# torognes/vsearch

Measured on AMD Instinct MI355X. Metric: GCUPS (useful DP cells/s of the search16 global-alignment path: DP + traceback + CIGAR), higher is better.
Workload: dtype int16

## Files before the change

include/vsx.h:

```cpp
#ifndef VSX_H
#define VSX_H

#include <stddef.h>
#include <stdint.h>

#ifdef __cplusplus
extern "C" {
#endif

#define VSX_API_VERSION 1000
#define VSX_SCORE_SENTINEL 32767

#define VSX_OK         0
#define VSX_EINVAL    -1
#define VSX_ENODEVICE -2
#define VSX_ENOMEM    -3
#define VSX_EHIP      -4

typedef struct vsx_ctx vsx_ctx;
typedef struct vsx_seqset vsx_seqset;
typedef struct vsx_plan vsx_plan;

typedef struct vsx_scoring {
  int64_t match;
// ... 47 lines not shown
  uint32_t traceback_launches;
  uint64_t cells;
  uint64_t dir_bytes;
} vsx_timing;

typedef struct vsx_plan_info {
  uint64_t tasks;
  uint64_t tasks_tilted;
  uint64_t tasks_tracked;
  uint32_t rows_dominant;
  uint32_t chunks;
  uint64_t tasks_max3;
  uint64_t tasks_sparse;
  uint64_t waves;
  uint64_t tasks_pair;
} vsx_plan_info;

const char * vsx_version_string(void);
int vsx_device_count(void);
const char * vsx_last_error(void);

int vsx_create(vsx_ctx ** out, const vsx_scoring * scoring, int device);
void vsx_destroy(vsx_ctx * ctx);


int vsx_seqset_create(vsx_ctx * ctx, vsx_seqset ** out, uint64_t n,
                      const char * blob, uint64_t blob_bytes,
                      const uint64_t * offsets, const uint32_t * lengths);
int vsx_seqset_create_from_device(vsx_ctx * ctx, vsx_seqset ** out, uint64_t n,
                                  const void * d_blob, uint64_t blob_bytes,
// ... 52 lines not shown
```

vsearch_amd/_lib.py:

```python
import ctypes as C
import os

HERE = os.path.dirname(os.path.abspath(__file__))
LIB_PATH = os.environ.get("VSX_LIBRARY") or os.path.join(HERE, "libvsx.so")

VSX_OK, VSX_EINVAL, VSX_ENODEVICE, VSX_ENOMEM, VSX_EHIP = 0, -1, -2, -3, -4
SENTINEL = 32767

SYMBOLS = [
    "vsx_version_string", "vsx_device_count", "vsx_last_error", "vsx_create", "vsx_destroy",
    "vsx_seqset_create", "vsx_seqset_create_both_strands", "vsx_seqset_create_from_device", "vsx_seqset_destroy", "vsx_seqset_count",
    "vsx_plan_create", "vsx_plan_run", "vsx_plan_sync", "vsx_plan_fetch", "vsx_plan_export_hits", "vsx_plan_export_runs",
    "vsx_cigar_from_runs", "vsx_plan_destroy",
    "vsx_align_pairs", "vsx_align_pairs_filtered", "vsx_align_pairs_ranked", "vsx_ranked_free", "vsx_plan_set_filter", "vsx_results_free", "vsx_plan_describe",
]
SEARCH_SYMBOLS = ["vsx_search_opts_default", "vsx_searcher_create", "vsx_searcher_destroy", "vsx_searcher_db_text", "vsx_search_batch",
                  "vsx_search_batch_meta", "vsx_searcher_set_meta",
                  "vsx_hits_free", "vsx_search_candidates", "vsx_search_candidates_batch", "vsx_candidates_free", "vsx_lma_align", "vsx_allpairs_block", "vsx_allpairs_rows", "vsx_allpairs_stream", "vsx_cluster_fast", "vsx_cluster_out_free", "vsx_msa", "vsx_msa_out_free",
                  "vsx_msa_device", "vsx_msa_device_batch", "vsx_dust_mask", "vsx_abundance_ratio_cmp",
                  "vsx_multi_searcher_create", "vsx_multi_searcher_destroy", "vsx_multi_searcher_devices", "vsx_multi_searcher_replica",
                  "vsx_multi_search_batch", "vsx_multi_allpairs",
                  "vsx_chimera_opts_default", "vsx_uchime_ref", "vsx_chimera_last_stats",
                  "vsx_chimera_denovo_opts_default", "vsx_uchime_denovo", "vsx_chimera_denovo_last_stats",
                  "vsx_chimeras_long_opts_default", "vsx_chimeras_denovo", "vsx_chimeras_denovo_last_stats",
# ... 191 lines not shown
                ("gaps", C.POINTER(C.c_uint16)), ("verdict", C.POINTER(C.c_uint8)), ("id", C.POINTER(C.c_double)),
                ("cigar_off", C.POINTER(C.c_uint64)), ("cigar_blob", C.POINTER(C.c_char)), ("cigar_bytes", C.c_uint64),
                ("n_undecided", C.c_uint64), ("undecided", C.POINTER(C.c_uint32))]


class Filter(C.Structure):
    _fields_ = [("iddef", C.c_int32), ("leftjust", C.c_int32), ("rightjust", C.c_int32), ("pad", C.c_int32),
                ("id", C.c_double), ("weak_id", C.c_double), ("maxid", C.c_double), ("mid", C.c_double),
                ("query_cov", C.c_double), ("target_cov", C.c_double),
                ("maxsubs", C.c_int64), ("maxgaps", C.c_int64), ("mincols", C.c_int64), ("maxdiffs", C.c_int64)]


class PlanInfo(C.Structure):
    _fields_ = [("tasks", C.c_uint64), ("tasks_tilted", C.c_uint64), ("tasks_tracked", C.c_uint64),
                ("rows_dominant", C.c_uint32), ("chunks", C.c_uint32), ("tasks_max3", C.c_uint64),
                ("tasks_sparse", C.c_uint64), ("waves", C.c_uint64), ("tasks_pair", C.c_uint64)]


class Timing(C.Structure):
    _fields_ = [("forward_ms", C.c_float), ("traceback_ms", C.c_float), ("total_ms", C.c_float),
                ("forward_launches", C.c_uint32), ("traceback_launches", C.c_uint32),
                ("cells", C.c_uint64), ("dir_bytes", C.c_uint64)]


class ClusterOut(C.Structure):
    _fields_ = [("n", C.c_uint64), ("n_clusters", C.c_uint64), ("clusterno", C.POINTER(C.c_uint32)), ("hits", Hits)]


class MsaOut(C.Structure):
    _fields_ = [("alnlen", C.c_uint64), ("n_rows", C.c_uint64), ("conslen", C.c_uint64), ("rows", C.POINTER(C.c_char)),
                ("consensus", C.POINTER(C.c_char)), ("profile", C.POINTER(C.c_uint64))]
# ... 125 lines not shown
```

vsearch_amd/csrc/ubench_d16.hip:

```cpp
#include <hip/hip_runtime.h>
#include <cstdio>
#include <cstdlib>

#define CK(x) do { hipError_t e = (x); if (e != hipSuccess) { fprintf(stderr, "%s:%d %s\n", __FILE__, __LINE__, hipGetErrorString(e)); exit(1); } } while (0)

__global__ void k_semantics(unsigned * out)
{
  __shared__ unsigned short tab[256];
  tab[threadIdx.x] = (unsigned short) (0x1100u + threadIdx.x);
  tab[threadIdx.x + 64] = (unsigned short) (0x2200u + threadIdx.x);
  __syncthreads();
  const unsigned addr = (unsigned) (size_t) tab + threadIdx.x * 2u;
  unsigned hi = 0xDEADBEEFu, lo = 0xDEADBEEFu, u16 = 0xDEADBEEFu;
  asm volatile("ds_read_u16_d16_hi %0, %3 offset:128\n"
               "ds_read_u16_d16 %1, %3\n"
               "ds_read_u16 %2, %3\n"
               "s_waitcnt lgkmcnt(0)\n" : "+v"(hi), "+v"(lo), "+v"(u16) : "v"(addr));
  out[threadIdx.x * 3 + 0] = hi;
  out[threadIdx.x * 3 + 1] = lo;
  out[threadIdx.x * 3 + 2] = u16;
}

typedef _Float16 f16x2 __attribute__((ext_vector_type(2)));
typedef unsigned short us2 __attribute__((ext_vector_type(2)));
// ... 53 lines not shown
        uint4 v4 = make_uint4(0, 0, 0, 0);
#pragma unroll
        for (int r = 0; r < R; ++r)
          {
            if ((r & 3) == 0) v4 = q4[r >> 2];
            const unsigned V = (r & 3) == 0 ? v4.x : ((r & 3) == 1 ? v4.y : ((r & 3) == 2 ? v4.z : v4.w));
            const unsigned h0 = Hd + V;
            const unsigned h2 = max3(h0, F, E[r]);
            Hd = hin[r];
            hout[r] = h2;
            const unsigned he = h2 - go;
            F = pmaxu(F, he);
            E[r] = pmaxu(E[r], he);
          }
      }
    else
      {
        const unsigned aA = (unsigned) (size_t) QP + (ca * (16 * R) + (unsigned) l * R) * 2u;
        const unsigned aB = (unsigned) (size_t) QP + (cb * (16 * R) + (unsigned) l * R) * 2u;
        unsigned lo[R], hi[R];
#define LOAD2(k) asm volatile("ds_read_u16 %0, %4 offset:%6\n ds_read_u16_d16_hi %1, %5 offset:%6\n ds_read_u16 %2, %4 offset:%7\n ds_read_u16_d16_hi %3, %5 offset:%7\n" \
                              : "=&v"(lo[2 * (k)]), "=&v"(hi[2 * (k)]), "=&v"(lo[2 * (k) + 1]), "=&v"(hi[2 * (k) + 1]) : "v"(aA), "v"(aB), "n"(4 * (k)), "n"(4 * (k) + 2))
#define WAIT2(k, n) asm volatile("s_waitcnt lgkmcnt(" #n ")" : "+v"(lo[2 * (k)]), "+v"(hi[2 * (k)]), "+v"(lo[2 * (k) + 1]), "+v"(hi[2 * (k) + 1]))
        LOAD2(0); LOAD2(1);
#pragma unroll
        for (int k = 0; k < R / 2; ++k)
          {
            if (k + 1 < R / 2) { WAIT2(k, 4); } else { WAIT2(k, 0); }
#pragma unroll
            for (int rr = 0; rr < 2; ++rr)
// ... 25 lines not shown
{
  const int blocks = 1024 * waves_per_simd, steps = 2000;
  unsigned * out; CK(hipMalloc(&out, (size_t) blocks * 64 * 4));
  hipEvent_t e0, e1; CK(hipEventCreate(&e0)); CK(hipEventCreate(&e1));
  hipLaunchKernelGGL(k_rows<MODE>, dim3(blocks), dim3(64), 0, 0, 20, out, 1u);
  CK(hipDeviceSynchronize());
  CK(hipEventRecord(e0));
  hipLaunchKernelGGL(k_rows<MODE>, dim3(blocks), dim3(64), 0, 0, steps, out, 1u);
  CK(hipEventRecord(e1));
  CK(hipEventSynchronize(e1));
  float ms; CK(hipEventElapsedTime(&ms, e0, e1));
  unsigned h0 = 0;
  CK(hipMemcpy(&h0, out, 4, hipMemcpyDeviceToHost));
  const double cycles = ms * 1e-3 * 2.4e9;
  printf("mode %d (%s) waves/SIMD %d: %8.3f ms, %.1f cycles per lane-row and wave   [check %08x]\n", MODE,
         MODE == 0 ? "b64 loads + perm, 6 VALU per row" : (MODE == 1 ? "u16 loads, add3, 5 VALU per row" : "pair profile, b128 loads, 5 VALU per row"), waves_per_simd, ms,
         cycles / ((double) steps * R * waves_per_simd), h0);
  CK(hipFree(out));
}

int main()
{
  hipDeviceProp_t p; CK(hipGetDeviceProperties(&p, 0));
  printf("device %s  CUs %d  arch %s\n", p.name, p.multiProcessorCount, p.gcnArchName);
  unsigned * out; CK(hipMalloc(&out, 64 * 3 * 4));
  hipLaunchKernelGGL(k_semantics, dim3(1), dim3(64), 0, 0, out);
  unsigned h[12]; CK(hipMemcpy(h, out, sizeof h, hipMemcpyDeviceToHost));
  printf("lane 0: d16_hi into 0xDEADBEEF -> %08x, d16 -> %08x, u16 -> %08x;  lane 1: %08x %08x %08x\n", h[0], h[1], h[2], h[3], h[4], h[5]);
  printf("  (table: lane x holds 0x1100 + x at its address, 0x2200 + x at +128)  d16_hi zeroes the low half: %s\n", (h[0] & 0xffffu) == 0 ? "YES" : "no");
  for (int w = 1; w <= 4; w *= 2) { run<0>(w); run<1>(w); if (w <= 2) run<2>(w); }
  run<0>(3);
  return 0;
}
```

vsearch_amd/csrc/vsx_device.hip:

```cpp
#include <hip/hip_runtime.h>
#include <type_traits>
#include <cstdlib>
#include <atomic>
#include "vsx_internal.h"

typedef unsigned int u32;
typedef unsigned int u32x4 __attribute__((ext_vector_type(4)));
typedef unsigned int u32x3 __attribute__((ext_vector_type(3)));
typedef short s2 __attribute__((ext_vector_type(2)));
typedef unsigned short us2 __attribute__((ext_vector_type(2)));

#define DEV __device__ __forceinline__
struct __attribute__((aligned(4))) Pair2 { unsigned int x, y; };

#define SIGN2 0x80008000u

DEV s2 S2(u32 x) { return __builtin_bit_cast(s2, x); }
DEV us2 U2(u32 x) { return __builtin_bit_cast(us2, x); }
DEV u32 UI(s2 x) { return __builtin_bit_cast(u32, x); }
DEV u32 UI(us2 x) { return __builtin_bit_cast(u32, x); }

DEV u32 sadd(u32 a, u32 b) { return UI(__builtin_elementwise_add_sat(S2(a), S2(b))); }
DEV u32 ssub(u32 a, u32 b) { return UI(__builtin_elementwise_sub_sat(S2(a), S2(b))); }
DEV u32 pmax(u32 a, u32 b) { return UI(__builtin_elementwise_max(S2(a), S2(b))); }
// ... 30 lines not shown
#ifndef VSX_FWD_WAVES
#define VSX_FWD_WAVES(R_, TILT_) ((R_) <= 16 ? 4 : ((R_) <= 24 ? 3 : 2))
#endif
#ifndef VSX_FWD_WAVES_ONE
#define VSX_FWD_WAVES_ONE(R_, TILT_) ((R_) == 26 ? 3 : VSX_FWD_WAVES(R_, TILT_))
#endif
typedef _Float16 f16x2 __attribute__((ext_vector_type(2)));
DEV u32 pk_max3_bits(u32 a, u32 b, u32 c)
{
  const f16x2 x = __builtin_bit_cast(f16x2, a), y = __builtin_bit_cast(f16x2, b), z = __builtin_bit_cast(f16x2, c);
  return __builtin_bit_cast(u32, __builtin_elementwise_maximum(__builtin_elementwise_maximum(x, y), z));
}
#ifndef VSX_FWD_WAVES_NQ
#define VSX_FWD_WAVES_NQ(R_, NQ_) ((NQ_) == 4 ? 2 : ((R_) <= 24 ? 3 : 2))
#endif
template <int R, bool TRACK, bool TILT = false, bool MAX3 = false, int NQ = 1, bool PAIR = false, bool ONE = false>
__global__ void __launch_bounds__(PAIR ? 256 : 64) __attribute__((amdgpu_waves_per_eu(NQ == 1 ? (ONE ? VSX_FWD_WAVES_ONE(R, TILT) : VSX_FWD_WAVES(R, TILT)) : VSX_FWD_WAVES_NQ(R, NQ), 8)))
vsx_forward_kernel(const VsxDevParams P, const VsxTask * __restrict__ tasks,
                   const uint8_t * __restrict__ qc, const uint8_t * __restrict__ tc,
                   u32 * __restrict__ dir, uint2 * strip, VsxSlotOut * __restrict__ slot_out, const u32 ntasks)
{
  constexpr bool TOPPAD = !TRACK;
  static_assert(!TILT || TOPPAD, "tilted coordinates exist for the TOPPAD class only");
  const int tl = TILT ? P.tilt : 0;
  static_assert(!MAX3 || TILT, "the MAX3 arithmetic is a sub-class of TILT");
  constexpr u32 BIAS16 = MAX3 ? 0x3E00u : (TILT ? 0x8000u : 0u);
  constexpr u32 BIAS = BIAS16 * 0x10001u;
  constexpr u32 CK_REBIAS = 0u;
  auto bpack = [](int v) -> u32 { return pack16(v + (int) BIAS16); };
  auto vadd = [](u32 a, u32 b) -> u32 { return TILT ? a + b : sadd(a, b); };
  auto vsubk = [](u32 a, u32 b) -> u32 { return TILT ? a - b : ssub(a, b); };
  auto vsub = [](u32 a, u32 b) -> u32 { return TILT ? psubw(a, b) : ssub(a, b); };
  auto vmax = [](u32 a, u32 b) -> u32 { return TILT ? pmaxu(a, b) : pmax(a, b); };
  constexpr bool MIDCK = VSX_MID(R, TILT);
  constexpr int RT = MIDCK ? R / 2 : R;
  constexpr bool QPL = TILT;
  constexpr int RP = (R + 3) & ~3;
  static_assert(NQ == 1 || NQ == 2 || NQ == 4, "tasks per wave");
  static_assert(NQ == 1 || TILT, "the sparse-task classes exist for the look-ahead TILT kernels only");
  static_assert(!PAIR || (NQ == 1 && TILT), "the pair-profile classes extend the FEED2 look-ahead kernels");
  constexpr int WPB = PAIR ? 4 : 1;
  constexpr int QPBYTES = 16 * 16 * RP;
  constexpr int RPP = ((RP / 4) & 1) ? RP : RP + 4;
  __shared__ __attribute__((aligned(16))) u32 PPf[PAIR ? 16 * 16 * RPP : 4];
  __shared__ __attribute__((aligned(16))) int16_t QP[!PAIR ? (QPL ? (NQ * QPBYTES) / 2 : 16 * 16 * R) : 8];
  constexpr int FSZ = (TILT ? 2 : 1) * 4 * 16;
  __shared__ uint4 FEED4a[FSZ * WPB];
  __shared__ u32 FEEDFa[FSZ * WPB];
  constexpr bool FEED2 = TILT;
  __shared__ uint2 FEEDBa[FEED2 ? 2 * 4 * 16 * WPB : 1];

  const int wv = PAIR ? __builtin_amdgcn_readfirstlane((int) (threadIdx.x >> 6)) : 0;
  uint4 * const FEED4 = FEED4a + wv * FSZ;
  u32 * const FEEDF = FEEDFa + wv * FSZ;
  uint2 * const FEEDB = FEEDBa + (FEED2 ? wv * FSZ : 0);
  const int lane = PAIR ? (int) (threadIdx.x & 63) : (int) threadIdx.x;
  const int gw = lane >> 4;
  constexpr int GPT = 4 / NQ;
  const int sq = (NQ == 1) ? 0 : gw / GPT;
  const int g = (NQ == 1) ? gw : gw % GPT;
  const int l = lane & 15;
  const u32 tix = PAIR ? blockIdx.x * 4u + (u32) wv : ((NQ == 1) ? blockIdx.x : blockIdx.x * (u32) NQ + (u32) sq);
  const bool sub_on = (NQ == 1 && !PAIR) ? true : (tix < ntasks);
  const VsxTask & T = tasks[sub_on ? tix : ntasks - 1];
  uint8_t * const QPl = reinterpret_cast<uint8_t *>(QP) + ((NQ == 1) ? 0 : sq * QPBYTES);

  const int Q = (int) T.qlen;
  const int total_lanes = (Q + R - 1) / R;
  const int rcnt0 = Q - (total_lanes - 1) * R;
  const int rc0 = __builtin_amdgcn_readfirstlane(rcnt0);
// ... 34 lines not shown
                  int va = 0, vb = 0;
                  if (rr < R)
                    {
                      if (Lr == 0 && rr < pad) va = vb = -P.top_step + 2 * tl;
                      else if (Lr < total_lanes)
                        {
                          const int gi = (Lr == 0) ? rr - pad : rcnt0 + (Lr - 1) * R + rr;
                          const int qs = (int) qq[gi];
                          va = P.matrix[(1 << (pr >> 2)) * 16 + qs];
                          vb = P.matrix[(1 << (pr & 3)) * 16 + qs];
                        }
                    }
                  PPf[(pr * 16 + row / RP) * RPP + rr] = ((u32) va & 0xffu) | (((u32) vb & 0xffu) << 16);
                }
            }
          else if (QPL)
            {
              constexpr int LPT = 64 / NQ;
              for (int idx = (NQ == 1) ? lane : lane % LPT; idx < 16 * 16 * RP; idx += LPT)
                {
                  const int code = idx / (16 * RP), row = idx % (16 * RP);
                  const int Lr = 16 * s + row / RP, rr = row % RP;
                  int v = 0;
                  if (rr < R)
                    {
                      if (Lr == 0 && rr < pad) v = -P.top_step + 2 * tl;
                      else if (Lr < total_lanes)
                        {
                          const int gi = (Lr == 0) ? rr - pad : rcnt0 + (Lr - 1) * R + rr;
                          v = P.matrix[code * 16 + (int) qq[gi]];
// ... 62 lines not shown
        rawA = (c < DA) ? (u32) tA[c] : 0u;
        rawB = (c < DB) ? (u32) tB[c] : 0u;
        if (s == 0) rawH = P.htop[c];
        else if (c < Dpg) rawS = strip_in[c];
      };
      prefetch(0);

      auto build_feed = [&](int blk, auto lean_tag) __attribute__((always_inline)) {
              constexpr bool LEAN = FEED2 && decltype(lean_tag)::value;
              const int c = 16 * blk + l;
              if (LEAN)
                {
                  f_H = (s == 0) ? bpack(rawH - pad * tl) : rawS.x;
                  f_F = (s == 0) ? vsub(f_H, qrt_i_pk) : rawS.y;
                  const u32 f_off = PAIR ? (((rawA >> 1) - (rawA >> 3)) * 4u + ((rawB >> 1) - (rawB >> 3))) * (u32) (16 * RPP * 4)
                                         : (rawA * (u32) (16 * RP) | ((rawB * (u32) (16 * RP)) << 16));
                  FEED4[(blk & 1) * 64 + gw * 16 + l] = make_uint4(f_off, 0u, f_H, f_F);
                  prefetch(blk + 1);
                  return;
                }
              const u32 qA = (u32) ((c < DA - 1) ? P.qrt_i : P.qrt_r) & 0xffffu;
              const u32 qB = (u32) ((c < DB - 1) ? P.qrt_i : P.qrt_r) & 0xffffu;
              const u32 rA = (u32) ((c < DA - 1) ? P.rt_i : P.rt_r) & 0xffffu;
              const u32 rB = (u32) ((c < DB - 1) ? P.rt_i : P.rt_r) & 0xffffu;
              const u32 sA = rawA | ((c == DA - 1) ? 0x100u : 0u) | ((c < DpA) ? 0x200u : 0u);
              const u32 sB = rawB | ((c == DB - 1) ? 0x100u : 0u) | ((c < DpB) ? 0x200u : 0u);
              f_sym = sA | (sB << 16);
              f_qrt = qA | (qB << 16);
              f_rt = rA | (rB << 16);
              if (s == 0)
                {
                  f_H = bpack(rawH - pad * tl);
                  f_F = vsub(f_H, f_qrt);
                }
              else
                {
                  f_H = rawS.x;
                  f_F = rawS.y;
                }
              const int fo = QPL ? (blk & 1) * 64 : 0;
              if (FEED2)
                {
                  const u32 f_off = PAIR ? (((rawA >> 1) - (rawA >> 3)) * 4u + ((rawB >> 1) - (rawB >> 3))) * (u32) (16 * RPP * 4)
                                         : (rawA * (u32) (16 * RP) | ((rawB * (u32) (16 * RP)) << 16));
                  FEED4[fo + gw * 16 + l] = make_uint4(f_off, f_sym, f_H, f_F);
                  FEEDB[fo + gw * 16 + l] = make_uint2(f_qrt, f_rt);
                }
              else
                {
                  FEED4[fo + gw * 16 + l] = make_uint4(f_sym, f_qrt, f_rt, f_H);
                  FEEDF[fo + gw * 16 + l] = f_F;
                }
              prefetch(blk + 1);
      };
      constexpr int PD = RP / 4;
      u32 profA[2][(QPL && !PAIR) ? PD : 1], profB[2][(QPL && !PAIR) ? PD : 1];
      auto load_profile = [&](u32 (&buf)[2][(QPL && !PAIR) ? PD : 1], u32 sy) __attribute__((always_inline)) {
        if (PAIR) return;
        const u32 cd = sy & 0x000F000Fu;
        constexpr int QPA = (RP % 16 == 0) ? 16 : ((RP % 8 == 0) ? 8 : 4);
        if (FEED2)
          {
            const uint8_t * pa = QPl + l * RP + (sy & 0xFFFFu);
            const uint8_t * pb = QPl + l * RP + (sy >> 16);
            constexpr int PDN = (QPL && !PAIR) ? PD : 1;
            if constexpr (PAIR) { }
            else if constexpr (QPA == 16)
              {
#pragma unroll
                for (int k = 0; k < PDN; k += 4)
                  {
                    const uint4 va = *reinterpret_cast<const uint4 *>(pa + 4 * k), vb = *reinterpret_cast<const uint4 *>(pb + 4 * k);
                    buf[0][k] = va.x; buf[0][k + 1] = va.y; buf[0][k + 2] = va.z; buf[0][k + 3] = va.w;
// ... 11 lines not shown
                  }
              }
            else
              {
#pragma unroll
                for (int k = 0; k < PDN; ++k)
                  { buf[0][k] = reinterpret_cast<const u32 *>(pa)[k]; buf[1][k] = reinterpret_cast<const u32 *>(pb)[k]; }
              }
            return;
          }
        const u32 * a = reinterpret_cast<const u32 *>(QPl + (cd & 0xFu) * (16 * RP) + l * RP);
        const u32 * b = reinterpret_cast<const u32 *>(QPl + (cd >> 16) * (16 * RP) + l * RP);
#pragma unroll
        for (int k = 0; k < ((QPL && !PAIR) ? PD : 1); ++k) { buf[0][k] = a[k]; buf[1][k] = b[k]; }
      };
      if (QPL)
        {
          build_feed(0, std::false_type {});
          sym = dpp_shr1(FEED4[gw * 16].x, 0u);
          load_profile(profA, sym);
        }

      const uint4 * const feed4_g = FEED4 + gw * 16;
      const u32 * const feedf_g = FEEDF + gw * 16;
      u32 pendH = 0, pendF = 0;
      u32 pendMH = 0, pendMF = 0, curMH = 0, curMF = 0;
      bool pend_on = false;
      const size_t ck_rowdw = ((((size_t) nstrips * steps + 1) & ~(size_t) 1) >> 1) * VSX_ROWCK_PAIR_DW(TILT);
      const size_t ck_nblk = ((size_t) steps + 15) >> 4;
      constexpr int CK_LANE_DW = TILT ? 3 : 4;
      constexpr size_t CK_COL_DW = TILT ? (size_t) 64 * 4 * VSX_COLCK_NB(R, true) : (size_t) 64 * (2 * R);
      const int ck_slot = VSX_CK_SLOT(TILT, gw, l);
      u32 * const rck_base = dir + T.dir_off + ((((size_t) s * steps) >> 1) * 64 + ck_slot) * CK_LANE_DW;
      u32 * const cck_base = dir + T.dir_off + ck_rowdw + (size_t) s * ck_nblk * CK_COL_DW;
      u32 * const mck_base = dir + T.dir_off + ck_rowdw + (size_t) nstrips * ck_nblk * CK_COL_DW
// ... 19 lines not shown
            }
          if (QPL) { if ((t & 15) == 15) build_feed((t >> 4) + 1, std::integral_constant<bool, LEANFEED> {}); }
          else if ((t & 15) == 0) build_feed(t >> 4, std::false_type {});

          const int fo = QPL ? ((t >> 4) & 1) * 64 : 0;
          const u32 fslot = (u32) (fo + (t & 15));
          const uint4 fv = feed4_g[fslot];
          const u32 fF = FEED2 ? fv.w : feedf_g[fslot];
          if (QPL)
            {
              const int t1 = t + 1;
              symn = dpp_shr1(feed4_g[(u32) (((t1 >> 4) & 1) * 64 + (t1 & 15))].x, sym);
              load_profile(pn, symn);
            }
          else sym = dpp_shr1(fv.x, sym);
          if (!INTERIOR)
            {
              if (FEED2)
                {
                  const uint2 fb = FEEDB[fo + gw * 16 + (t & 15)];
                  qrt = dpp_shr1(fb.x, qrt); rt = dpp_shr1(fb.y, rt);
                  symf = dpp_shr1(fv.y, symf);
                }
              else { qrt = dpp_shr1(fv.y, qrt); rt = dpp_shr1(fv.z, rt); }
            }
          const u32 inH = dpp_shr1(FEED2 ? fv.z : fv.w, outH);
          const u32 inF = dpp_shr1(fF, outF);

          const int j = t - l;
          const bool active = STEADY ? true : (lane_on && j >= 0 && j < Dpg);
          if (active)
            {
              const u32 code = sym & 0x000F000Fu;
              const int16_t * qpA = QP + (code & 0xFu) * (16 * R) + l * R;
              const int16_t * qpB = QP + (code >> 16) * (16 * R) + l * R;
              u32 pa = 0, pb = 0;
              u32 Hd = diag;
              u32 F = inF;
              u32 smn = 0x7FFF7FFFu, smx = 0x80008000u;
              u32 h2 = 0;
              u32 capH = 0, capF = 0, capmn = 0, capmx = 0;
              u32 lastL = 0, lastEL = 0;
              u32 midH = 0, midF = 0;
              auto rows = [&](auto shared_tag) __attribute__((always_inline)) {
              constexpr bool SHARED = decltype(shared_tag)::value;
              constexpr bool LASTFAST = MAX3 && SHARED;
#pragma unroll
              for (int r = 0; r < R; ++r)
                {
                  u32 V;
                  if (PAIR) V = pp[r];
                  else if (QPL)
                    {
                      if ((r & 3) == 0) { pa = pc[0][r >> 2]; pb = pc[1][r >> 2]; }
                      V = __builtin_amdgcn_perm(pb, pa, 0x0C040C00u + 0x00010001u * (u32) (r & 3));
                    }
                  else
                    {
                      if (R % 2 == 0)
                        {
                          if ((r & 3) == 0 && r + 3 < R)
                            {
                              typedef typename std::conditional<R % 4 == 0, uint2, Pair2>::type Rows4;
                              const Rows4 va = *reinterpret_cast<const Rows4 *>(qpA + r);
                              const Rows4 vb = *reinterpret_cast<const Rows4 *>(qpB + r);
                              pa = va.x; pb = vb.x;
                              ac[r + 1] = va.y; ac[r + 2] = vb.y;
                            }
                          else if ((r & 3) == 0)
                            {
                              pa = *reinterpret_cast<const u32 *>(qpA + r);
                              pb = *reinterpret_cast<const u32 *>(qpB + r);
                            }
                          else if ((r & 3) == 2) { pa = ac[r - 1]; pb = ac[r]; }
                          V = (r & 1) ? __builtin_amdgcn_perm(pb, pa, 0x07060302u) : __builtin_amdgcn_perm(pb, pa, 0x05040100u);
                        }
                      else V = (u32) (uint16_t) qpA[r] | ((u32) (uint16_t) qpB[r] << 16);
                    }
                  const u32 h0 = vadd(Hd, V);
                  const bool ONE_MAX = MAX3 && (r < R - 1 || LASTFAST);
                  const u32 h1 = ONE_MAX ? 0u : vmax(h0, F);
                  h2 = ONE_MAX ? pk_max3_bits(h0, F, E[r]) : vmax(h1, E[r]);
                  if (TRACK) { smn = pmin(smn, h2); smx = pmax(smx, h2); }
                  Hd = hin[r];
                  hout[r] = h2;
                  const u32 qrq = (r == R - 1) ? qrq_last : P.qrq_i_pk;
                  const u32 rq = (r == R - 1) ? rq_last : P.rq_i_pk;
                  const u32 he = (r < R - 1) ? vsubk(h2, qrq) : vsub(h2, qrq);
                  const u32 hf = (SHARED && r < R - 1) ? he : vsub(h2, qrt);
                  const u32 f = (TILT && INTERIOR) ? F : vsub(F, rt);
                  const u32 e = (TILT && INTERIOR && r < R - 1) ? E[r] : vsub(E[r], rq);
                  if (r == R - 1) { lastL = LASTFAST ? 0u : vsub(h1, E[r]); lastEL = vsub(he, e); }
                  F = vmax(f, hf);
                  E[r] = vmax(e, he);
// ... 1400 lines not shown
static hipError_t launch_fwd2(int track, int nq, int one, const VsxDevParams & P, const VsxTask * d_tasks, uint32_t ntasks,
                              const uint8_t * q, const uint8_t * t, uint32_t * dir, uint2 * strip,
                              VsxSlotOut * slot, hipStream_t st)
{
  if (nq == 8)
    {
      if (!(P.tilt != 0 && !track) || (ntasks & 3u)) return hipErrorInvalidValue;
      if constexpr (R >= 4)
        {
          if (!one) return hipErrorInvalidValue;
          if (P.max3) VSX_FWD_GO4(ntasks / 4, R, false, true, true, 1, true, true); else VSX_FWD_GO4(ntasks / 4, R, false, true, false, 1, true, true);
          return hipGetLastError();
        }
      else return hipErrorInvalidValue;
    }
  if (nq != 1)
    {
      if (!(P.tilt != 0 && !track && (nq == 2 || nq == 4))) return hipErrorInvalidValue;
      if constexpr (R >= 4)
        {
          const uint32_t grid = (ntasks + (uint32_t) nq - 1) / (uint32_t) nq;
          if (nq == 2) { if (P.max3) VSX_FWD_GO(grid, R, false, true, true, 2); else VSX_FWD_GO(grid, R, false, true, false, 2); }
          else         { if (P.max3) VSX_FWD_GO(grid, R, false, true, true, 4); else VSX_FWD_GO(grid, R, false, true, false, 4); }
          return hipGetLastError();
        }
      else return hipErrorInvalidValue;
    }
  if (P.tilt != 0)
    {
      if (track) return hipErrorInvalidValue;
// ... 95 lines not shown
```

vsearch_amd/csrc/vsx_host.cpp:

```cpp
#include "../../include/vsx.h"
#include "vsx_internal.h"
#include "vsx_private.h"

#include <hip/hip_runtime.h>
#include <algorithm>
#include <cinttypes>
#include <cstdio>
#include <cstdlib>
#include <cstring>
#include <sched.h>
#include <thread>
#include <atomic>
#include <condition_variable>
#include <mutex>
#include <chrono>
#include <deque>
#include <functional>
#include <memory>
#include <numeric>
#include <string>
#include <vector>

using vsxp::fail;
using vsxp::DevBuf;
// ... 885 lines not shown
  {
    std::vector<uint64_t> bad((size_t) nthc, UINT64_MAX);
    auto check = [&](int t) {
      const uint64_t lo = n_pairs * (uint64_t) t / (uint64_t) nthc, hi = n_pairs * (uint64_t) (t + 1) / (uint64_t) nthc;
      for (uint64_t k = lo; k < hi; ++k)
        if (qidx[k] >= queries->n || tidx[k] >= targets->n) { bad[(size_t) t] = k; return; }
    };
    run_threads(nthc, check);
    for (int t = 0; t < nthc; ++t)
      if (bad[(size_t) t] != UINT64_MAX)
        return fail(VSX_EINVAL, "vsx_plan_create: pair %" PRIu64 " references a sequence out of range", bad[(size_t) t]);
  }
  VSX_HIP(hipSetDevice(ctx->device));
  static const bool pair_env = std::getenv("VSX_PAIRPROF") ? std::strcmp(std::getenv("VSX_PAIRPROF"), "0") != 0 : (VSX_PAIRPROF_DEFAULT != 0);
  const bool pair_try = pair_env && n_pairs >= 32;

  std::unique_ptr<vsx_plan> pl(new vsx_plan);
  pl->ctx = ctx; pl->Q = queries; pl->T = targets; pl->n_pairs = n_pairs;
  {
    std::lock_guard<std::mutex> lk(ctx->slot_mu);
    const unsigned seq = ctx->plan_seq.fetch_add(1);
    int pick = -1;
    for (int k = 0; k < 3; ++k)
      if (ctx->slot_refs[k] == 0 && (pick < 0 || ctx->shared_dir[k].bytes() > ctx->shared_dir[pick].bytes())) pick = k;
    if (pick < 0)
      for (int k = 0; k < 3; ++k)
        if (pick < 0 || (int) (seq - ctx->slot_stamp[k]) > (int) (seq - ctx->slot_stamp[pick])) pick = k;
    ++ctx->slot_refs[pick];
    ctx->slot_stamp[pick] = seq;
    pl->dir_slot = pick;
// ... 205 lines not shown
      std::vector<Key> ks;
      for (const ProtoTask & pt : protos)
        {
          if (pt.nq != 2 && pt.nq != 4) continue;
          bool found = false;
          for (Key & c : ks) if (c.rows == pt.rows && c.track == pt.track && c.tilt == pt.tilt && c.nq == pt.nq) { ++c.count; found = true; break; }
          if (!found) ks.push_back(Key {pt.rows, pt.track, pt.tilt, pt.nq, 1});
        }
      bool any = false;
      for (const Key & c : ks) any = any || c.count < sparse_min;
      if (any)
        for (ProtoTask & pt : protos)
          if (pt.nq == 2 || pt.nq == 4)
            for (const Key & c : ks)
              if (c.count < sparse_min && pt.nq == c.nq && pt.rows == c.rows && pt.track == c.track && pt.tilt == c.tilt) { pt.nq = 1; break; }
    }
  auto by_class = [](const ProtoTask & a, const ProtoTask & b) {
    if (a.rows != b.rows) return a.rows < b.rows;
    if (a.track != b.track) return a.track < b.track;
    if (a.tilt != b.tilt) return a.tilt < b.tilt;
    return a.nq < b.nq;
  };
  if (!std::is_sorted(protos.begin(), protos.end(), by_class)) std::stable_sort(protos.begin(), protos.end(), by_class);

  double t_budget = 0;
  if (dir_budget_bytes == 0)
    {
      size_t free_b = 0, total_b = 0;
      const double tb0 = now();
      VSX_HIP(hipMemGetInfo(&free_b, &total_b));
// ... 248 lines not shown
  VSX_HIP(hipMemsetAsync(pl->d_cursor.p, 0, 2 * sizeof(unsigned long long), st));
  if (pl->filter.rank_counts) VSX_HIP(hipMemsetAsync(pl->d_rank_counts.p, 0, 2 * sizeof(uint32_t), st));
  VSX_HIP(hipEventRecord(pl->ev_begin, st));
  for (size_t k = 0; k < pl->chunks.size(); ++k)
    {
      Chunk & c = pl->chunks[k];
      uint32_t * dir = pl->d_dir[0].p;
      if (k >= 1) VSX_HIP(hipStreamWaitEvent(st, pl->chunks[k - 1].e2, 0));
      else if (ctx->ev_tb_used[slot]) VSX_HIP(hipStreamWaitEvent(st, ctx->ev_tb[slot], 0));
      VSX_HIP(hipEventRecord(c.e0, st));
      for (const Launch & L : c.launches)
        {
          VsxDevParams Pf = L.tilt ? ctx->Pt : ctx->P;
          Pf.max3 = (L.tilt == 2) ? 1 : 0;
          static const bool one_off = std::getenv("VSX_ONESTRIP") && std::strcmp(std::getenv("VSX_ONESTRIP"), "0") == 0;
          VSX_HIP(vsx_launch_forward(L.rows, L.track, L.nq, (L.multi || (one_off && L.nq != 8)) ? 0 : 1, Pf, pl->d_tasks.p + L.first, L.count,
                                    pl->Q->codes(), pl->T->codes(), dir, pl->d_strip.p,
                                    pl->d_slot.p + (size_t) L.first * VSX_TASK_SLOTS, st));
        }
      VSX_HIP(hipEventRecord(c.e1, st));
      VSX_HIP(hipStreamWaitEvent(st2, c.e1, 0));
      VSX_HIP(hipEventRecord(c.e1b, st2));
      for (size_t li = 0; li < c.launches.size();)
        {
          const Launch & L = c.launches[li];
          uint32_t pair_count = L.pair_count;
          size_t lj = li + 1;
          while (lj < c.launches.size() && c.launches[lj].rows == L.rows &&
                 c.launches[lj].track == L.track && c.launches[lj].tilt == L.tilt) { pair_count += c.launches[lj].pair_count; ++lj; }
          VsxDevParams Pb = L.tilt ? ctx->Pt : ctx->P;
          Pb.max3 = (L.tilt == 2) ? 1 : 0;
// ... 43 lines not shown
  return VSX_OK;
}

int vsx_plan_describe(const vsx_plan * pl, vsx_plan_info * info)
{
  if (!pl || !info) return fail(VSX_EINVAL, "vsx_plan_describe: null argument");
  *info = vsx_plan_info {};
  info->tasks = pl->tasks.size();
  info->chunks = (uint32_t) pl->chunks.size();
  uint64_t best = 0;
  for (const Chunk & c : pl->chunks)
    for (const Launch & L : c.launches)
      {
        if (L.nq == 2 || L.nq == 4) info->tasks_sparse += L.count;
        if (L.nq == 8) info->tasks_pair += L.count;
        info->waves += (L.nq == 2 || L.nq == 4) ? (L.count + (uint32_t) L.nq - 1) / (uint32_t) L.nq : L.count;
        if (L.tilt) info->tasks_tilted += L.count;
        if (L.tilt == 2) info->tasks_max3 += L.count;
        if (L.track) info->tasks_tracked += L.count;
        if (L.count > best) { best = L.count; info->rows_dominant = (uint32_t) L.rows; }
      }
  return VSX_OK;
}

static void append_cigar(std::string & s, const uint32_t * runs, uint32_t n)
{
  static const char ops[4] = {'M', 'I', 'D', '?'};
  char buf[16];
  for (uint32_t k = n; k-- > 0;)
    {
// ... 547 lines not shown
```

vsearch_amd/csrc/vsx_internal.h:

```cpp
#ifndef VSX_INTERNAL_H
#define VSX_INTERNAL_H

#include <stdint.h>
#include <hip/hip_runtime_api.h>

#define VSX_TASK_SLOTS 8
#define VSX_GROUP_LANES 16
#define VSX_MAX_SEQLEN_SUM 65535LL
#define VSX_MAX_SEQLEN_PRODUCT 25000000LL
#define VSX_TABLE_LEN (65536 + 64)
#define VSX_CODE_SLACK 64
#define VSX_CK_SLACK_DW 4096
#ifndef VSX_MID_MIN_ROWS
#define VSX_MID_MIN_ROWS 18
#endif
#define VSX_MID(R_, TILT_) ((TILT_) && (R_) >= VSX_MID_MIN_ROWS)

struct VsxDevParams {
  uint32_t match_pk;
  uint32_t qrq_i_pk, rq_i_pk;
  uint32_t qrq_r_pk, rq_r_pk;
  int32_t  qrt_i, rt_i;
  int32_t  qrt_r, rt_r;
  int32_t  match, mismatch;
  int32_t  smin;
  int32_t  n_mismatch;
  int32_t  share_sub;
  int32_t  top_open, top_step;
  int32_t  tilt;
  int32_t  max3;
  const int16_t * htop;
// ... 166 lines not shown
```

Measured before the change: 8208.

## Add split LO/HI query-profile forward kernel class for pure MAX3 single-strip tasks

```diff
diff --git a/include/vsx.h b/include/vsx.h
--- a/include/vsx.h
+++ b/include/vsx.h
@@ -85,6 +85,7 @@
   uint64_t tasks_sparse;
   uint64_t waves;
   uint64_t tasks_pair;
+  uint64_t tasks_split;
 } vsx_plan_info;
 
 const char * vsx_version_string(void);
diff --git a/vsearch_amd/_lib.py b/vsearch_amd/_lib.py
--- a/vsearch_amd/_lib.py
+++ b/vsearch_amd/_lib.py
@@ -229,7 +229,8 @@
 class PlanInfo(C.Structure):
     _fields_ = [("tasks", C.c_uint64), ("tasks_tilted", C.c_uint64), ("tasks_tracked", C.c_uint64),
                 ("rows_dominant", C.c_uint32), ("chunks", C.c_uint32), ("tasks_max3", C.c_uint64),
-                ("tasks_sparse", C.c_uint64), ("waves", C.c_uint64), ("tasks_pair", C.c_uint64)]
+                ("tasks_sparse", C.c_uint64), ("waves", C.c_uint64), ("tasks_pair", C.c_uint64),
+                ("tasks_split", C.c_uint64)]
 
 
 class Timing(C.Structure):
diff --git a/vsearch_amd/csrc/ubench_d16.hip b/vsearch_amd/csrc/ubench_d16.hip
--- a/vsearch_amd/csrc/ubench_d16.hip
+++ b/vsearch_amd/csrc/ubench_d16.hip
@@ -91,6 +91,34 @@
             E[r] = pmaxu(E[r], he);
           }
       }
+    else if (MODE == 3)
+      {
+        const char * base = reinterpret_cast<const char *>(QP) + l * 16;
+        const char * pa = base + (ca & 3u) * 1024u, * pb = base + ((cb & 3u) + 4u) * 1024u;
+        uint4 lo = *reinterpret_cast<const uint4 *>(pa), hi = *reinterpret_cast<const uint4 *>(pb), lo2, hi2;
+#pragma unroll
+        for (int r = 0; r < R; ++r)
+          {
+            if ((r & 3) == 0)
+              {
+                if (r) { lo = lo2; hi = hi2; }
+                const int k = (r >> 2) + 1;
+                if (k < R / 4) { lo2 = *reinterpret_cast<const uint4 *>(pa + k * 256); hi2 = *reinterpret_cast<const uint4 *>(pb + k * 256); }
+                else { lo2 = *reinterpret_cast<const uint4 *>(base + (cb & 3u) * 1024u); hi2 = *reinterpret_cast<const uint4 *>(base + ((ca & 3u) + 4u) * 1024u); }
+              }
+            const unsigned vl = (r & 3) == 0 ? lo.x : ((r & 3) == 1 ? lo.y : ((r & 3) == 2 ? lo.z : lo.w));
+            const unsigned vh = (r & 3) == 0 ? hi.x : ((r & 3) == 1 ? hi.y : ((r & 3) == 2 ? hi.z : hi.w));
+            const unsigned h0 = Hd + vl + vh;
+            const unsigned h2 = max3(h0, F, E[r]);
+            Hd = hin[r];
+            hout[r] = h2;
+            const unsigned he = h2 - go;
+            F = pmaxu(F, he);
+            E[r] = pmaxu(E[r], he);
+          }
+        Hd ^= lo2.x & hi2.x & 1u;
+        diag ^= Hd & 1u;
+      }
     else
       {
         const unsigned aA = (unsigned) (size_t) QP + (ca * (16 * R) + (unsigned) l * R) * 2u;
@@ -146,7 +174,7 @@
   CK(hipMemcpy(&h0, out, 4, hipMemcpyDeviceToHost));
   const double cycles = ms * 1e-3 * 2.4e9;
   printf("mode %d (%s) waves/SIMD %d: %8.3f ms, %.1f cycles per lane-row and wave   [check %08x]\n", MODE,
-         MODE == 0 ? "b64 loads + perm, 6 VALU per row" : (MODE == 1 ? "u16 loads, add3, 5 VALU per row" : "pair profile, b128 loads, 5 VALU per row"), waves_per_simd, ms,
+         MODE == 0 ? "b64 loads + perm, 6 VALU per row" : (MODE == 1 ? "u16 loads, add3, 5 VALU per row" : (MODE == 2 ? "pair profile, b128 loads, 5 VALU per row" : "split LO / HI tables, 2 x b128 per 4 rows, add3, 5 VALU per row")), waves_per_simd, ms,
          cycles / ((double) steps * R * waves_per_simd), h0);
   CK(hipFree(out));
 }
@@ -162,5 +190,6 @@
   printf("  (table: lane x holds 0x1100 + x at its address, 0x2200 + x at +128)  d16_hi zeroes the low half: %s\n", (h[0] & 0xffffu) == 0 ? "YES" : "no");
   for (int w = 1; w <= 4; w *= 2) { run<0>(w); run<1>(w); if (w <= 2) run<2>(w); }
   run<0>(3);
+  run<3>(4); run<3>(3);
   return 0;
 }
diff --git a/vsearch_amd/csrc/vsx_device.hip b/vsearch_amd/csrc/vsx_device.hip
--- a/vsearch_amd/csrc/vsx_device.hip
+++ b/vsearch_amd/csrc/vsx_device.hip
@@ -68,7 +68,7 @@
 #ifndef VSX_FWD_WAVES_NQ
 #define VSX_FWD_WAVES_NQ(R_, NQ_) ((NQ_) == 4 ? 2 : ((R_) <= 24 ? 3 : 2))
 #endif
-template <int R, bool TRACK, bool TILT = false, bool MAX3 = false, int NQ = 1, bool PAIR = false, bool ONE = false>
+template <int R, bool TRACK, bool TILT = false, bool MAX3 = false, int NQ = 1, bool PAIR = false, bool ONE = false, bool SPLIT = false>
 __global__ void __launch_bounds__(PAIR ? 256 : 64) __attribute__((amdgpu_waves_per_eu(NQ == 1 ? (ONE ? VSX_FWD_WAVES_ONE(R, TILT) : VSX_FWD_WAVES(R, TILT)) : VSX_FWD_WAVES_NQ(R, NQ), 8)))
 vsx_forward_kernel(const VsxDevParams P, const VsxTask * __restrict__ tasks,
                    const uint8_t * __restrict__ qc, const uint8_t * __restrict__ tc,
@@ -93,21 +93,25 @@
   static_assert(NQ == 1 || NQ == 2 || NQ == 4, "tasks per wave");
   static_assert(NQ == 1 || TILT, "the sparse-task classes exist for the look-ahead TILT kernels only");
   static_assert(!PAIR || (NQ == 1 && TILT), "the pair-profile classes extend the FEED2 look-ahead kernels");
+  static_assert(!SPLIT || (TILT && MAX3 && NQ == 1 && !PAIR && ONE), "the split-profile classes are whole-wave single-strip MAX3 kernels");
   constexpr int WPB = PAIR ? 4 : 1;
   constexpr int QPBYTES = 16 * 16 * RP;
   constexpr int RPP = ((RP / 4) & 1) ? RP : RP + 4;
   __shared__ __attribute__((aligned(16))) u32 PPf[PAIR ? 16 * 16 * RPP : 4];
-  __shared__ __attribute__((aligned(16))) int16_t QP[!PAIR ? (QPL ? (NQ * QPBYTES) / 2 : 16 * 16 * R) : 8];
+  constexpr int NQT = RP / 4;
+  static_assert(!SPLIT || NQT >= 2, "the split-profile rows are read a quarter ahead");
+  constexpr int SPSYM = NQT * 256;
+  __shared__ __attribute__((aligned(16))) int16_t QP[!PAIR ? (SPLIT ? (2 * 4 * SPSYM) / 2 : (QPL ? (NQ * QPBYTES) / 2 : 16 * 16 * R)) : 8];
   constexpr int FSZ = (TILT ? 2 : 1) * 4 * 16;
   __shared__ uint4 FEED4a[FSZ * WPB];
   __shared__ u32 FEEDFa[FSZ * WPB];
   constexpr bool FEED2 = TILT;
-  __shared__ uint2 FEEDBa[FEED2 ? 2 * 4 * 16 * WPB : 1];
+  __shared__ uint2 FEEDBa[(FEED2 && !SPLIT) ? 2 * 4 * 16 * WPB : 1];
 
   const int wv = PAIR ? __builtin_amdgcn_readfirstlane((int) (threadIdx.x >> 6)) : 0;
   uint4 * const FEED4 = FEED4a + wv * FSZ;
   u32 * const FEEDF = FEEDFa + wv * FSZ;
-  uint2 * const FEEDB = FEEDBa + (FEED2 ? wv * FSZ : 0);
+  uint2 * const FEEDB = FEEDBa + ((FEED2 && !SPLIT) ? wv * FSZ : 0);
   const int lane = PAIR ? (int) (threadIdx.x & 63) : (int) threadIdx.x;
   const int gw = lane >> 4;
   constexpr int GPT = 4 / NQ;
@@ -172,6 +176,26 @@
                   PPf[(pr * 16 + row / RP) * RPP + rr] = ((u32) va & 0xffu) | (((u32) vb & 0xffu) << 16);
                 }
             }
+          else if (SPLIT)
+            {
+              u32 * const TAB = reinterpret_cast<u32 *>(QP);
+              for (int idx = lane; idx < 2 * 4 * NQT * 64; idx += 64)
+                {
+                  const int tb = idx / (4 * NQT * 64), sy = (idx / (NQT * 64)) & 3, k = (idx % (NQT * 64)) >> 6;
+                  const int Lr = (idx >> 2) & 15, rr = 4 * k + (idx & 3);
+                  int v = 0;
+                  if (rr < R)
+                    {
+                      if (Lr == 0 && rr < pad) v = -P.top_step + 2 * tl;
+                      else if (Lr < total_lanes)
+                        {
+                          const int gi = (Lr == 0) ? rr - pad : rcnt0 + (Lr - 1) * R + rr;
+                          v = P.matrix[(1 << sy) * 16 + (int) qq[gi]];
+                        }
+                    }
+                  TAB[idx] = ((u32) v & 0xffu) << (tb ? 16 : 0);
+                }
+            }
           else if (QPL)
             {
               constexpr int LPT = 64 / NQ;
@@ -264,6 +288,7 @@
                   f_H = (s == 0) ? bpack(rawH - pad * tl) : rawS.x;
                   f_F = (s == 0) ? vsub(f_H, qrt_i_pk) : rawS.y;
                   const u32 f_off = PAIR ? (((rawA >> 1) - (rawA >> 3)) * 4u + ((rawB >> 1) - (rawB >> 3))) * (u32) (16 * RPP * 4)
+                                  : SPLIT ? (((rawA >> 1) - (rawA >> 3)) * (u32) SPSYM | ((((rawB >> 1) - (rawB >> 3)) + 4u) * (u32) SPSYM) << 16)
                                          : (rawA * (u32) (16 * RP) | ((rawB * (u32) (16 * RP)) << 16));
                   FEED4[(blk & 1) * 64 + gw * 16 + l] = make_uint4(f_off, 0u, f_H, f_F);
                   prefetch(blk + 1);
@@ -273,8 +298,8 @@
               const u32 qB = (u32) ((c < DB - 1) ? P.qrt_i : P.qrt_r) & 0xffffu;
               const u32 rA = (u32) ((c < DA - 1) ? P.rt_i : P.rt_r) & 0xffffu;
               const u32 rB = (u32) ((c < DB - 1) ? P.rt_i : P.rt_r) & 0xffffu;
-              const u32 sA = rawA | ((c == DA - 1) ? 0x100u : 0u) | ((c < DpA) ? 0x200u : 0u);
-              const u32 sB = rawB | ((c == DB - 1) ? 0x100u : 0u) | ((c < DpB) ? 0x200u : 0u);
+              const u32 sA = rawA | ((c == DA - 1) ? 0x100u : 0u) | ((c < DpA) ? 0x200u : 0u) | ((SPLIT && !(c < DA - 1)) ? 0x400u : 0u);
+              const u32 sB = rawB | ((c == DB - 1) ? 0x100u : 0u) | ((c < DpB) ? 0x200u : 0u) | ((SPLIT && !(c < DB - 1)) ? 0x400u : 0u);
               f_sym = sA | (sB << 16);
               f_qrt = qA | (qB << 16);
               f_rt = rA | (rB << 16);
@@ -292,9 +317,10 @@
               if (FEED2)
                 {
                   const u32 f_off = PAIR ? (((rawA >> 1) - (rawA >> 3)) * 4u + ((rawB >> 1) - (rawB >> 3))) * (u32) (16 * RPP * 4)
+                                  : SPLIT ? (((rawA >> 1) - (rawA >> 3)) * (u32) SPSYM | ((((rawB >> 1) - (rawB >> 3)) + 4u) * (u32) SPSYM) << 16)
                                          : (rawA * (u32) (16 * RP) | ((rawB * (u32) (16 * RP)) << 16));
                   FEED4[fo + gw * 16 + l] = make_uint4(f_off, f_sym, f_H, f_F);
-                  FEEDB[fo + gw * 16 + l] = make_uint2(f_qrt, f_rt);
+                  if (!SPLIT) FEEDB[fo + gw * 16 + l] = make_uint2(f_qrt, f_rt);
                 }
               else
                 {
@@ -306,7 +332,7 @@
       constexpr int PD = RP / 4;
       u32 profA[2][(QPL && !PAIR) ? PD : 1], profB[2][(QPL && !PAIR) ? PD : 1];
       auto load_profile = [&](u32 (&buf)[2][(QPL && !PAIR) ? PD : 1], u32 sy) __attribute__((always_inline)) {
-        if (PAIR) return;
+        if (PAIR || SPLIT) return;
         const u32 cd = sy & 0x000F000Fu;
         constexpr int QPA = (RP % 16 == 0) ? 16 : ((RP % 8 == 0) ? 8 : 4);
         if (FEED2)
@@ -348,11 +374,20 @@
 #pragma unroll
         for (int k = 0; k < ((QPL && !PAIR) ? PD : 1); ++k) { buf[0][k] = a[k]; buf[1][k] = b[k]; }
       };
+      u32 sq0l[4] = {0, 0, 0, 0}, sq0h[4] = {0, 0, 0, 0};
+      const uint8_t * const sp_lane = reinterpret_cast<const uint8_t *>(QP) + l * 16;
+      auto split_read = [&](u32 * lo, u32 * hi, u32 sy, int k) __attribute__((always_inline)) {
+        const uint4 va = *reinterpret_cast<const uint4 *>(sp_lane + (sy & 0xFFFFu) + k * 256);
+        const uint4 vb = *reinterpret_cast<const uint4 *>(sp_lane + (sy >> 16) + k * 256);
+        lo[0] = va.x; lo[1] = va.y; lo[2] = va.z; lo[3] = va.w;
+        hi[0] = vb.x; hi[1] = vb.y; hi[2] = vb.z; hi[3] = vb.w;
+      };
       if (QPL)
         {
           build_feed(0, std::false_type {});
           sym = dpp_shr1(FEED4[gw * 16].x, 0u);
           load_profile(profA, sym);
+          if (SPLIT) split_read(sq0l, sq0h, sym, 0);
         }
 
       const uint4 * const feed4_g = FEED4 + gw * 16;
@@ -402,13 +437,25 @@
               load_profile(pn, symn);
             }
           else sym = dpp_shr1(fv.x, sym);
+          u32 sc0l[4], sc0h[4];
+#pragma unroll
+          for (int z = 0; z < 4; ++z) { sc0l[z] = sq0l[z]; sc0h[z] = sq0h[z]; }
+          if (SPLIT && !STEADY) split_read(sq0l, sq0h, symn, 0);
           if (!INTERIOR)
             {
               if (FEED2)
                 {
-                  const uint2 fb = FEEDB[fo + gw * 16 + (t & 15)];
-                  qrt = dpp_shr1(fb.x, qrt); rt = dpp_shr1(fb.y, rt);
                   symf = dpp_shr1(fv.y, symf);
+                  if (SPLIT)
+                    {
+                      const u32 em = a_pk_ashr15(symf << 5);
+                      qrt = a_bfi_v(em, pack16(P.qrt_r), qrt_i_pk); rt = a_bfi_v(em, pack16(P.rt_r), pack16(P.rt_i));
+                    }
+                  else
+                    {
+                      const uint2 fb = FEEDB[fo + gw * 16 + (t & 15)];
+                      qrt = dpp_shr1(fb.x, qrt); rt = dpp_shr1(fb.y, rt);
+                    }
                 }
               else { qrt = dpp_shr1(fv.y, qrt); rt = dpp_shr1(fv.z, rt); }
             }
@@ -423,6 +470,13 @@
               const int16_t * qpA = QP + (code & 0xFu) * (16 * R) + l * R;
               const int16_t * qpB = QP + (code >> 16) * (16 * R) + l * R;
               u32 pa = 0, pb = 0;
+              u32 spl[SPLIT ? RP : 1], sph[SPLIT ? RP : 1];
+              if (SPLIT)
+                {
+#pragma unroll
+                  for (int z = 0; z < 4; ++z) { spl[SPLIT ? z : 0] = sc0l[z]; sph[SPLIT ? z : 0] = sc0h[z]; }
+                  if (NQT > 1) split_read(spl + (SPLIT ? 4 : 0), sph + (SPLIT ? 4 : 0), sym, 1);
+                }
               u32 Hd = diag;
               u32 F = inF;
               u32 smn = 0x7FFF7FFFu, smx = 0x80008000u;
@@ -436,8 +490,16 @@
 #pragma unroll
               for (int r = 0; r < R; ++r)
                 {
-                  u32 V;
-                  if (PAIR) V = pp[r];
+                  u32 V = 0;
+                  if (SPLIT)
+                    {
+                      if ((r & 3) == 0 && r > 0)
+                        {
+                          if (r / 4 + 1 < NQT) split_read(spl + (SPLIT ? r + 4 : 0), sph + (SPLIT ? r + 4 : 0), sym, r / 4 + 1);
+                          else if (STEADY) split_read(sq0l, sq0h, symn, 0);
+                        }
+                    }
+                  else if (PAIR) V = pp[r];
                   else if (QPL)
                     {
                       if ((r & 3) == 0) { pa = pc[0][r >> 2]; pb = pc[1][r >> 2]; }
@@ -465,7 +527,7 @@
                         }
                       else V = (u32) (uint16_t) qpA[r] | ((u32) (uint16_t) qpB[r] << 16);
                     }
-                  const u32 h0 = vadd(Hd, V);
+                  const u32 h0 = SPLIT ? Hd + spl[SPLIT ? r : 0] + sph[SPLIT ? r : 0] : vadd(Hd, V);
                   const bool ONE_MAX = MAX3 && (r < R - 1 || LASTFAST);
                   const u32 h1 = ONE_MAX ? 0u : vmax(h0, F);
                   h2 = ONE_MAX ? pk_max3_bits(h0, F, E[r]) : vmax(h1, E[r]);
@@ -1896,6 +1958,16 @@
         }
       else return hipErrorInvalidValue;
     }
+  if (nq == 16)
+    {
+      if (!(P.tilt != 0 && P.max3 && !track && one)) return hipErrorInvalidValue;
+      if constexpr (VSX_SPLIT_ROWS(R))
+        {
+          VSX_FWD_GO(ntasks, R, false, true, true, 1, false, true, true);
+          return hipGetLastError();
+        }
+      else return hipErrorInvalidValue;
+    }
   if (nq != 1)
     {
       if (!(P.tilt != 0 && !track && (nq == 2 || nq == 4))) return hipErrorInvalidValue;
diff --git a/vsearch_amd/csrc/vsx_host.cpp b/vsearch_amd/csrc/vsx_host.cpp
--- a/vsearch_amd/csrc/vsx_host.cpp
+++ b/vsearch_amd/csrc/vsx_host.cpp
@@ -923,6 +923,7 @@
   VSX_HIP(hipSetDevice(ctx->device));
   static const bool pair_env = std::getenv("VSX_PAIRPROF") ? std::strcmp(std::getenv("VSX_PAIRPROF"), "0") != 0 : (VSX_PAIRPROF_DEFAULT != 0);
   const bool pair_try = pair_env && n_pairs >= 32;
+  static const bool split_env = !(std::getenv("VSX_SPLITPROF") && std::strcmp(std::getenv("VSX_SPLITPROF"), "0") == 0);
 
   std::unique_ptr<vsx_plan> pl(new vsx_plan);
   pl->ctx = ctx; pl->Q = queries; pl->T = targets; pl->n_pairs = n_pairs;
@@ -1158,6 +1159,31 @@
           if (pt.nq == 2 || pt.nq == 4)
             for (const Key & c : ks)
               if (c.count < sparse_min && pt.nq == c.nq && pt.rows == c.rows && pt.track == c.track && pt.tilt == c.tilt) { pt.nq = 1; break; }
+    }
+  if (split_env)
+    {
+      auto split_shape = [&](const ProtoTask & pt) {
+        return pt.nq == 1 && pt.tilt == 2 && VSX_SPLIT_ROWS(pt.rows) && (int64_t) queries->len[pt.q] <= 16ll * pt.rows;
+      };
+      bool any = false;
+      for (size_t x = 0; x < protos.size() && !any; ++x) any = split_shape(protos[x]);
+      if (any)
+        {
+          const int rc = ensure_impure(targets);
+          if (rc != VSX_OK) return rc;
+          const int nts = (int) std::max<size_t>(1, std::min<size_t>((size_t) vsx_internal_usable_cpus(), protos.size() / 4096));
+          run_threads(nts, [&](int th) {
+            const size_t lo = protos.size() * (size_t) th / (size_t) nts, hi = protos.size() * (size_t) (th + 1) / (size_t) nts;
+            for (size_t x = lo; x < hi; ++x)
+              {
+                ProtoTask & pt = protos[x];
+                if (!split_shape(pt)) continue;
+                bool pure = true;
+                for (uint32_t sidx = 0; sidx < pt.n && pure; ++sidx) pure = !targets->impure[tidx[pt.pair[sidx]]];
+                if (pure) pt.nq = 16;
+              }
+          });
+        }
     }
   auto by_class = [](const ProtoTask & a, const ProtoTask & b) {
     if (a.rows != b.rows) return a.rows < b.rows;
@@ -1436,7 +1462,7 @@
           VsxDevParams Pf = L.tilt ? ctx->Pt : ctx->P;
           Pf.max3 = (L.tilt == 2) ? 1 : 0;
           static const bool one_off = std::getenv("VSX_ONESTRIP") && std::strcmp(std::getenv("VSX_ONESTRIP"), "0") == 0;
-          VSX_HIP(vsx_launch_forward(L.rows, L.track, L.nq, (L.multi || (one_off && L.nq != 8)) ? 0 : 1, Pf, pl->d_tasks.p + L.first, L.count,
+          VSX_HIP(vsx_launch_forward(L.rows, L.track, L.nq, (L.multi || (one_off && L.nq < 8)) ? 0 : 1, Pf, pl->d_tasks.p + L.first, L.count,
                                     pl->Q->codes(), pl->T->codes(), dir, pl->d_strip.p,
                                     pl->d_slot.p + (size_t) L.first * VSX_TASK_SLOTS, st));
         }
@@ -1510,6 +1536,7 @@
       {
         if (L.nq == 2 || L.nq == 4) info->tasks_sparse += L.count;
         if (L.nq == 8) info->tasks_pair += L.count;
+        if (L.nq == 16) info->tasks_split += L.count;
         info->waves += (L.nq == 2 || L.nq == 4) ? (L.count + (uint32_t) L.nq - 1) / (uint32_t) L.nq : L.count;
         if (L.tilt) info->tasks_tilted += L.count;
         if (L.tilt == 2) info->tasks_max3 += L.count;
diff --git a/vsearch_amd/csrc/vsx_internal.h b/vsearch_amd/csrc/vsx_internal.h
--- a/vsearch_amd/csrc/vsx_internal.h
+++ b/vsearch_amd/csrc/vsx_internal.h
@@ -15,6 +15,7 @@
 #define VSX_MID_MIN_ROWS 18
 #endif
 #define VSX_MID(R_, TILT_) ((TILT_) && (R_) >= VSX_MID_MIN_ROWS)
+#define VSX_SPLIT_ROWS(R_) ((R_) == 10 || (R_) == 16)
 
 struct VsxDevParams {
   uint32_t match_pk;
```

New measurement: 8348, median of 6. 1.7% higher.
